# Hagtaril/HiddenPose

Hardware: AMD Instinct MI355X
Metric: samples/sec (128x128x512 meas) fwd+bwd (higher is better)
Workload: dtype f32; 1 GPU; NlosPose train step (fwd+L2Joint+BCEDice loss+bwd+Adam), 128x128x512 transients, batch 4/GPU, fp32, random-init weights, weight gradients of the 3^3 / 4^3 convolutions (and of small 1^3 ones) on a second stream; global_batch=4, world_size=1, parallelism=dp1

## Files before the change

### hiddenpose_amd/csrc/conv_kernels.hip

```cpp
#include <algorithm>
#include <cstdlib>
#include <cstring>
#include <mutex>
#include <type_traits>
#include <vector>

#include "hp_internal.h"

namespace hp {

using f32x16 = __attribute__((ext_vector_type(16))) float;
using bf16x8 = __attribute__((ext_vector_type(8))) __bf16;
using bf16x4 = __attribute__((ext_vector_type(4))) __bf16;
using bf16x2 = __attribute__((ext_vector_type(2))) __bf16;
using f32x2 = __attribute__((ext_vector_type(2))) float;
using s16x4 = __attribute__((ext_vector_type(4))) short;

__device__ __forceinline__ bf16x4 to_bf16x4(const float4 v) {
  const bf16x2 lo = __builtin_convertvector((f32x2){v.x, v.y}, bf16x2);
  const bf16x2 hi = __builtin_convertvector((f32x2){v.z, v.w}, bf16x2);
  return (bf16x4){lo[0], lo[1], hi[0], hi[1]};
}

enum IgemmMode { MODE_CONV = 0, MODE_DECONV = 1, MODE_DGRAD_S2K3 = 2, MODE_STEM = 3 };
// ... 2247 lines not shown
      const float* pl = ring + ((z + a - 3) & 7) * SF_PLANE + (2 * wave) * SF_RX + lane;
#pragma unroll
      for (int bb = 0; bb < 7; ++bb) {
        const float* wt = wl + ((a * 7 + bb) * 7) * 64 + sub * 16;
#pragma unroll
        for (int c = 0; c < 7; ++c) {
          float wr[16];
#pragma unroll
          for (int q = 0; q < 4; ++q) {
            const f32x4c t4 = *(const f32x4c*)(wt + c * 64 + 4 * q);
            wr[4 * q] = t4[0];
            wr[4 * q + 1] = t4[1];
            wr[4 * q + 2] = t4[2];
            wr[4 * q + 3] = t4[3];
          }
#pragma unroll
          for (int r = 0; r < 2; ++r) {
            const float xv = pl[(r + bb) * SF_RX + c];
#pragma unroll
            for (int cg = 0; cg < 16; ++cg) acc[r][cg] = __builtin_amdgcn_mfma_f32_4x4x1f32(wr[cg], xv, acc[r][cg], 0, 0, 0);
          }
        }
      }
    }
#pragma unroll
    for (int r = 0; r < 2; ++r) {
      const int oy = y0 + 2 * wave + r;
      const bool row_ok = oy < H;
      const long orow = (((long)b * D + z) * H + oy) * W + x0;
#pragma unroll
      for (int hh = 0; hh < 2; ++hh) {
#pragma unroll
        for (int cg = 0; cg < 8; ++cg)
#pragma unroll
          for (int i = 0; i < 4; ++i) ot[lane * 33 + cg * 4 + i] = acc[r][8 * hh + cg][i];
        if (row_ok) {
          if (stats && lane < 32) {
            float s = 0.f, q = 0.f;
            const int nv = min(64, W - x0);
            for (int v = 0; v < nv; ++v) {
              const float val = ot[v * 33 + lane];
              s += val;
              q += val * val;
            }
            ssum[hh] += s;
            ssq[hh] += q;
          }
          const int q4 = lane & 7;
#pragma unroll
          for (int it = 0; it < 8; ++it) {
            const int v = it * 8 + (lane >> 3);
            if (x0 + v < W) {
              const float* sp = ot + v * 33 + 4 * q4;
              *(float4*)(Y + (orow + v) * 64 + 32 * hh + 4 * q4) = make_float4(sp[0], sp[1], sp[2], sp[3]);
            }
          }
        }
      }
    }
    if (z + 1 < ze) stage_store(z + 4, nv);
    __syncthreads();
  }
  if (stats && lane < 32) {
#pragma unroll
    for (int hh = 0; hh < 2; ++hh) {
      double* const slot = stats + (size_t)(blockIdx.x & (HP_STATS_SLOTS - 1)) * 128;
      atomicAdd(slot + 32 * hh + lane, (double)ssum[hh]);
      atomicAdd(slot + 64 + 32 * hh + lane, (double)ssq[hh]);
    }
  }
}

__global__ void k_pack_weight(const float* __restrict__ w, float* __restrict__ out, int Cout, int Cin, int taps,
                              int transposed, int swap, int to_torch) {
  const long total = (long)Cout * Cin * taps;
  for (long i = (long)blockIdx.x * blockDim.x + threadIdx.x; i < total; i += (long)gridDim.x * blockDim.x) {
    const int inner = (int)(i % (swap ? Cout : Cin));
    long r = i / (swap ? Cout : Cin);
    const int outer = (int)(r % (swap ? Cin : Cout));
    const int t = (int)(r / (swap ? Cin : Cout));
    const int co = swap ? inner : outer, ci = swap ? outer : inner;
    const long ti = transposed ? ((long)ci * Cout + co) * taps + t : ((long)co * Cin + ci) * taps + t;
    if (to_torch)
      ((float*)w)[ti] = out[i];
    else
      out[i] = w[ti];
  }
}

__global__ __launch_bounds__(256) void k_pack_weight_tiled(const float* __restrict__ w, float* __restrict__ out, int Cout,
                                                           int Cin, int taps, int transposed, int swap, int to_torch,
                                                           int out_half = 0) {
  __shared__ float tile[64][65];
  const int A = swap ? Cin : Cout, Bn = swap ? Cout : Cin;
  const int a = blockIdx.y, bn0 = blockIdx.x * 64;
  const int nb = min(64, Bn - bn0), n = nb * taps;
  auto torch_index = [&](int bn, int t) -> long {
    const int co = swap ? bn : a, ci = swap ? a : bn;
    return transposed ? ((long)ci * Cout + co) * taps + t : ((long)co * Cin + ci) * taps + t;
  };
  if (!to_torch) {
    for (int e = threadIdx.x; e < n; e += 256) {
      const int bl = e / taps, t = e - bl * taps;
      tile[bl][t] = w[torch_index(bn0 + bl, t)];
    }
    __syncthreads();
    for (int e = threadIdx.x; e < taps * 64; e += 256) {
      const int t = e >> 6, bl = e & 63;
      if (bl < nb) hp_st1(out, ((long)t * A + a) * Bn + bn0 + bl, tile[bl][t], out_half);
    }
  } else {
    for (int e = threadIdx.x; e < taps * 64; e += 256) {
      const int t = e >> 6, bl = e & 63;
      if (bl < nb) tile[bl][t] = out[((long)t * A + a) * Bn + bn0 + bl];
    }
    __syncthreads();
    for (int e = threadIdx.x; e < n; e += 256) {
      const int bl = e / taps, t = e - bl * taps;
      ((float*)w)[torch_index(bn0 + bl, t)] = tile[bl][t];
    }
  }
}

__global__ void k_pack_stem(const float* __restrict__ w, float* __restrict__ out, int Cout, int kpad, int to_torch) {
  const long total = (long)Cout * kpad;
  for (long i = (long)blockIdx.x * blockDim.x + threadIdx.x; i < total; i += (long)gridDim.x * blockDim.x) {
    const int k = (int)(i % kpad), n = (int)(i / kpad);
    if (to_torch) {
      if (k < 343) ((float*)w)[(long)n * 343 + k] = out[i];
    } else {
      out[i] = k < 343 ? w[(long)n * 343 + k] : 0.f;
    }
  }
}

struct ConvPlan {
  IgemmGeom fwd, dgrad, wgrad;
  int fwd_classes = 1, dgrad_classes = 1, wgrad_tapsum = 1;
  bool stem = false, dgrad_zero_fill = false;
  int planes = 0;
};

static void set_shifts(IgemmGeom& g) {
  g.sw = g.sh = g.sd = -1;
  if (g.mode >= 0 && is_pow2(g.gw) && is_pow2(g.gh) && is_pow2(g.gd) && g.M < (1l << 32)) {
    g.sw = ilog2(g.gw);
    g.sh = ilog2(g.gh);
    g.sd = ilog2(g.gd);
  }
}

static int make_plan(const hp_conv_desc& d, ConvPlan& p) {
  HP_REQUIRE(d.B >= 1 && d.Cin >= 1 && d.Cout >= 1, "conv: bad channel/batch sizes");
  HP_REQUIRE(d.precision >= HP_PRECISION_FP32 && d.precision <= HP_PRECISION_BF16X6, "conv: unknown precision %d", d.precision);
  HP_REQUIRE(d.io == 0 || d.precision == HP_PRECISION_BF16, "conv: bf16 activation tensors (io = %d) go with HP_PRECISION_BF16", d.io);
  p.planes = d.precision;
  const int k = d.k, s = d.stride, pad = d.pad;
  IgemmGeom f{};
  if (!d.transposed) {
    const int Do = (d.Di + 2 * pad - k) / s + 1, Ho = (d.Hi + 2 * pad - k) / s + 1, Wo = (d.Wi + 2 * pad - k) / s + 1;
    p.stem = (d.Cin == 1 && k == 7 && s == 1 && pad == 3);
    if (!p.stem) HP_REQUIRE(d.Cin % 4 == 0, "conv: Cin must be a multiple of 4 (got %d)", d.Cin);
    HP_REQUIRE(s == 1 || s == 2, "conv: stride must be 1 or 2");
    const int kpt = p.stem ? (343 + 31) / 32 : (d.Cin + 31) / 32;
    f = IgemmGeom{p.stem ? MODE_STEM : MODE_CONV, d.B, d.Di, d.Hi, d.Wi, d.Cin, Do, Ho, Wo, d.Cout, Do, Ho, Wo, 1,
                  k, s, pad, 0, (long)d.B * Do * Ho * Wo, kpt};
    p.fwd = f;
    p.fwd_classes = 1;
    p.wgrad = f;
    p.wgrad_tapsum = p.stem ? 1 : k * k * k;
    IgemmGeom g{};
    if (p.stem) {
      g = IgemmGeom{MODE_CONV, d.B, Do, Ho, Wo, d.Cout, d.Di, d.Hi, d.Wi, 1, d.Di, d.Hi, d.Wi, 1,
                    7, 1, 3, 1, (long)d.B * d.Di * d.Hi * d.Wi, d.Cout / 32};
      p.dgrad_classes = 1;
    } else if (s == 1) {
      HP_REQUIRE(d.Cout % 4 == 0, "conv dgrad: Cout must be a multiple of 4 (got %d)", d.Cout);
      g = IgemmGeom{MODE_CONV, d.B, Do, Ho, Wo, d.Cout, d.Di, d.Hi, d.Wi, d.Cin, d.Di, d.Hi, d.Wi, 1,
                    k, 1, pad, 1, (long)d.B * d.Di * d.Hi * d.Wi, (d.Cout + 31) / 32};
      p.dgrad_classes = 1;
    } else if (k == 3 && pad == 1) {
      HP_REQUIRE(d.Di % 2 == 0 && d.Hi % 2 == 0 && d.Wi % 2 == 0 && d.Cout % 32 == 0, "conv dgrad s2: even dims needed");
      g = IgemmGeom{MODE_DGRAD_S2K3, d.B, Do, Ho, Wo, d.Cout, d.Di, d.Hi, d.Wi, d.Cin, d.Di / 2, d.Hi / 2, d.Wi / 2, 2,
                    3, 1, 1, 0, (long)d.B * (d.Di / 2) * (d.Hi / 2) * (d.Wi / 2), d.Cout / 32};
      p.dgrad_classes = 8;
    } else if (k == 1 && pad == 0) {
      HP_REQUIRE(d.Di % 2 == 0 && d.Hi % 2 == 0 && d.Wi % 2 == 0 && d.Cout % 32 == 0, "conv dgrad s2: even dims needed");
      g = IgemmGeom{MODE_CONV, d.B, Do, Ho, Wo, d.Cout, d.Di, d.Hi, d.Wi, d.Cin, Do, Ho, Wo, 2,
                    1, 1, 0, 0, (long)d.B * Do * Ho * Wo, d.Cout / 32};
      p.dgrad_classes = 1;
      p.dgrad_zero_fill = true;
    } else {
      set_error("conv: unsupported stride-2 kernel %d pad %d", k, pad);
      return HP_ERR_UNSUPPORTED;
    }
    p.dgrad = g;
  } else {
    HP_REQUIRE(k == 4 && s == 2 && pad == 1, "deconv: only k4 s2 p1 is supported");
    HP_REQUIRE(d.Cin % 32 == 0 && d.Cout % 32 == 0, "deconv: channels must be multiples of 32");
    const int Do = 2 * d.Di, Ho = 2 * d.Hi, Wo = 2 * d.Wi;
    f = IgemmGeom{MODE_DECONV, d.B, d.Di, d.Hi, d.Wi, d.Cin, Do, Ho, Wo, d.Cout, d.Di, d.Hi, d.Wi, 2,
                  4, 1, 1, 0, (long)d.B * d.Di * d.Hi * d.Wi, d.Cin / 32};
    p.fwd = f;
    p.fwd_classes = 8;
    p.wgrad = f;
    p.wgrad_tapsum = 64;
    p.dgrad = IgemmGeom{MODE_CONV, d.B, Do, Ho, Wo, d.Cout, d.Di, d.Hi, d.Wi, d.Cin, d.Di, d.Hi, d.Wi, 1,
                        4, 2, 1, 0, (long)d.B * d.Di * d.Hi * d.Wi, d.Cout / 32};
    p.dgrad_classes = 1;
  }
  HP_REQUIRE((long)d.B * d.Di * d.Hi * d.Wi * (d.transposed ? 8 : 1) < (1l << 31), "conv: more than 2^31 voxels per tensor");
  set_shifts(p.fwd);
  set_shifts(p.dgrad);
  set_shifts(p.wgrad);
  p.fwd.welems = p.wgrad.welems = p.stem ? (long)d.Cout * ((343 + 31) / 32 * 32) : (long)d.Cout * d.Cin * k * k * k;
  p.dgrad.welems = (long)d.Cout * d.Cin * k * k * k;
  return HP_OK;
}

template <bool STEM, bool STATS, int NP, bool XH = false>
static void launch_igemm_bn(const IgemmGeom& g, int classes, const void* X, const float* W, const float* bias, void* Y,
                            double* stats, const void* addend, const unsigned char* amask, hipStream_t st) {
  if constexpr (NP == 1 && !STEM && !XH) {
    if (g.xh && g.Cin % 64 == 0) return launch_igemm_bn<STEM, STATS, NP, true>(g, classes, X, W, bias, Y, stats, addend, amask, st);
  }
  const unsigned mt = (unsigned)((g.M + BM - 1) / BM);
  static const bool gl_on = !(getenv("HP_IGEMM_GL") && atoi(getenv("HP_IGEMM_GL")) == 0);
  const bool gl = XH && g.wh && gl_on;
  static const bool bl_on = !(getenv("HP_IGEMM_BL") && atoi(getenv("HP_IGEMM_BL")) == 0);
  const bool bl = !XH && !g.xh && !g.wh && !STEM && bl_on && g.Cin % 32 == 0 && (long)g.Nout * g.Cin * class_ntaps(g, 0) * 4 * (g.mode == MODE_DECONV ? 8 : 1) < (1l << 31);
  static const bool slab_on = !(getenv("HP_IGEMM_SLAB") && atoi(getenv("HP_IGEMM_SLAB")) == 0);
  if (slab_on && g.Nout <= 64) {
    IgemmGeom gs = g;
    gs.slab = (int)((mt + 7) / 8);
    const dim3 grid((mt + 7) / 8 * 8, 1, classes);
    if constexpr (!XH && !STEM) {
      if (bl && g.Nout > 32) {
        hipLaunchKernelGGL((k_igemm<64, false, STATS, NP, false, false, true>), grid, dim3(CT), 0, st, X, W, bias, Y, stats, addend, amask, gs);
        return;
      }
    }
  }
  if (g.Nout > 64) {
    const unsigned tn = (unsigned)((g.Nout + 127) / 128);
    IgemmGeom gg = g;
    gg.tn = tn > 1 ? (int)tn : 0;
    gg.slab = slab_on ? (int)((mt + 7) / 8) : 0;
    const dim3 grid = (tn > 1 || gg.slab) ? dim3((mt + 7) / 8 * 8 * (tn > 1 ? tn : 1), 1, classes) : dim3(mt, 1, classes);
    if constexpr (XH) {
      if (gl) {
        hipLaunchKernelGGL((k_igemm<128, STEM, STATS, NP, true, true>), grid, dim3(CT), 0, st, X, W, bias, Y, stats, addend, amask, gg);
        return;
      }
    }
    if constexpr (!XH && !STEM) {
      if (bl) {
        hipLaunchKernelGGL((k_igemm<128, false, STATS, NP, false, false, true>), grid, dim3(CT), 0, st, X, W, bias, Y, stats, addend, amask, gg);
        return;
      }
    }
    hipLaunchKernelGGL((k_igemm<128, STEM, STATS, NP, XH>), grid, dim3(CT), 0, st, X, W, bias, Y, stats, addend, amask, gg);
  } else if (g.Nout > 32) {
    if constexpr (XH) {
      if (gl) {
        hipLaunchKernelGGL((k_igemm<64, STEM, STATS, NP, true, true>), dim3(mt, 1, classes), dim3(CT), 0, st, X, W, bias, Y, stats, addend, amask, g);
        return;
      }
    }
    if constexpr (!XH && !STEM) {
      if (bl) {
        hipLaunchKernelGGL((k_igemm<64, false, STATS, NP, false, false, true>), dim3(mt, 1, classes), dim3(CT), 0, st, X, W, bias, Y, stats, addend, amask, g);
        return;
      }
    }
    hipLaunchKernelGGL((k_igemm<64, STEM, STATS, NP, XH>), dim3(mt, 1, classes), dim3(CT), 0, st, X, W, bias, Y, stats, addend, amask, g);
  } else {
    hipLaunchKernelGGL((k_igemm<32, STEM, STATS, NP, XH>), dim3(mt, 1, classes), dim3(CT), 0, st, X, W, bias, Y, stats, addend, amask, g);
  }
}

template <int NP>
static void launch_igemm_p(const IgemmGeom& g, int classes, bool stem, const void* X, const float* W, const float* bias,
                           void* Y, double* stats, const void* addend, const unsigned char* amask, hipStream_t st) {
  if (stem) {
    if (stats) launch_igemm_bn<true, true, NP>(g, classes, X, W, bias, Y, stats, addend, amask, st);
    else launch_igemm_bn<true, false, NP>(g, classes, X, W, bias, Y, stats, addend, amask, st);
  } else {
    if (stats) launch_igemm_bn<false, true, NP>(g, classes, X, W, bias, Y, stats, addend, amask, st);
    else launch_igemm_bn<false, false, NP>(g, classes, X, W, bias, Y, stats, addend, amask, st);
  }
}

static void launch_igemm(const IgemmGeom& g, int classes, bool stem, int planes, const void* X, const float* W,
                         const float* bias, void* Y, double* stats, const void* addend, hipStream_t st,
                         const unsigned char* amask = nullptr) {
  switch (planes) {
    case 1: launch_igemm_p<1>(g, classes, stem, X, W, bias, Y, stats, addend, amask, st); break;
    case 2: launch_igemm_p<2>(g, classes, stem, X, W, bias, Y, stats, addend, amask, st); break;
    case 3: launch_igemm_p<3>(g, classes, stem, X, W, bias, Y, stats, addend, amask, st); break;
    default: launch_igemm_p<0>(g, classes, stem, X, W, bias, Y, stats, addend, amask, st); break;
  }
}

}

using namespace hp;

extern "C" size_t hp_conv3d_packed_weight_elems(const hp_conv_desc* d) {
  if (!d) return 0;
  if (!d->transposed && d->Cin == 1 && d->k == 7) return (size_t)d->Cout * ((343 + 31) / 32 * 32);
  return (size_t)d->Cout * d->Cin * d->k * d->k * d->k;
}

extern "C" int hp_conv3d_pack_weight(const hp_conv_desc* d, const float* w_torch, void* w_fwd_v, void* w_dgrad_v,
                                     void* stream) {
  float* const w_fwd = (float*)w_fwd_v;
  float* const w_dgrad = (float*)w_dgrad_v;
  HP_REQUIRE(d && w_torch, "hp_conv3d_pack_weight: null argument");
  ConvPlan p;
  int rc = make_plan(*d, p);
  if (rc) return rc;
  hipStream_t st = (hipStream_t)stream;
  const int taps = d->k * d->k * d->k;
  if (p.stem) {
    const int kpad = p.fwd.kpt * BK;
    HP_PROF("conv_pack_weight", st);
    if (w_fwd) hipLaunchKernelGGL(k_pack_stem, dim3(64), dim3(256), 0, st, w_torch, w_fwd, d->Cout, kpad, 0);
    if (w_dgrad) hipLaunchKernelGGL(k_pack_weight, dim3(64), dim3(256), 0, st, w_torch, w_dgrad, d->Cout, 1, 343, 0, 1, 0);
  } else {
    HP_REQUIRE(taps <= 64, "conv: at most 64 taps (got %d)", taps);
    HP_PROF("conv_pack_weight", st);
    const int wh = (d->io & HP_IO_W_BF16) ? 1 : 0;
    if (w_fwd)
      hipLaunchKernelGGL(k_pack_weight_tiled, dim3((d->Cin + 63) / 64, d->Cout), dim3(256), 0, st, w_torch, w_fwd, d->Cout,
                         d->Cin, taps, d->transposed, 0, 0, wh);
    if (w_dgrad)
      hipLaunchKernelGGL(k_pack_weight_tiled, dim3((d->Cout + 63) / 64, d->Cin), dim3(256), 0, st, w_torch, w_dgrad, d->Cout,
                         d->Cin, taps, d->transposed, 1, 0, wh);
  }
  HP_CHECK_HIP(hipGetLastError());
  return HP_OK;
}

extern "C" int hp_conv3d_unpack_wgrad(const hp_conv_desc* d, const float* dw_packed, float* dw_torch, void* stream) {
  HP_REQUIRE(d && dw_packed && dw_torch, "hp_conv3d_unpack_wgrad: null argument");
  ConvPlan p;
  int rc = make_plan(*d, p);
  if (rc) return rc;
  hipStream_t st = (hipStream_t)stream;
  const int taps = d->k * d->k * d->k;
  HP_PROF("conv_pack_weight", st);
  if (p.stem) {
    hipLaunchKernelGGL(k_pack_stem, dim3(64), dim3(256), 0, st, dw_torch, (float*)dw_packed, d->Cout, p.fwd.kpt * BK, 1);
  } else {
    hipLaunchKernelGGL(k_pack_weight_tiled, dim3((d->Cin + 63) / 64, d->Cout), dim3(256), 0, st, dw_torch, (float*)dw_packed,
                       d->Cout, d->Cin, taps, d->transposed, 0, 1);
  }
  HP_CHECK_HIP(hipGetLastError());
  return HP_OK;
}

extern "C" int hp_conv3d_forward(const hp_conv_desc* d, const void* x, const float* w_fwd, const float* bias, void* y,
                                 double* stats, void* stream) {
  HP_REQUIRE(d && x && w_fwd && y, "hp_conv3d_forward: null argument");
  ConvPlan p;
  int rc = make_plan(*d, p);
  if (rc) return rc;
  HP_REQUIRE(!(p.stem && (d->io & HP_IO_X_BF16)), "hp_conv3d_forward: the stem reads its single-channel input as fp32");
  p.fwd.xh = (d->io & HP_IO_X_BF16) ? 1 : 0;
  p.fwd.yh = (d->io & HP_IO_Y_BF16) ? 1 : 0;
  p.fwd.wh = (d->io & HP_IO_W_BF16) ? 1 : 0;
  HP_REQUIRE(!p.fwd.wh || (p.fwd.xh && p.planes == 1 && !p.stem && d->Cin % 64 == 0),
             "hp_conv3d_forward: bf16 packed weights go with a bf16 input, HP_PRECISION_BF16 and Cin %% 64 == 0");
  hipStream_t st = (hipStream_t)stream;
  if (stats) HP_CHECK_HIP(hipMemsetAsync(stats, 0, sizeof(double) * 2 * d->Cout * HP_STATS_SLOTS, st));
  if (p.stem && p.planes == 1 && d->Cout == 64 && !bias && !p.fwd.yh) {
    const int pz = (d->Di + SFH_TZ - 1) / SFH_TZ, py = (d->Hi + SFH_TY - 1) / SFH_TY, px = (d->Wi + SFH_TX - 1) / SFH_TX;
    const long tiles = (long)d->B * pz * py * px;
    const int per_wg = (int)std::max<long>(1, (tiles + 511) / 512);
    const size_t lds = sizeof(__bf16) * (SFH_W + 4 * SFH_COPY) + sizeof(float) * 8 * 64 * 2;
    static std::once_flag lds_once_h;
    static hipError_t lds_rc_h = hipSuccess;
    std::call_once(lds_once_h, [&] {
      lds_rc_h = hipFuncSetAttribute((const void*)k_stem_fwd_bf16, hipFuncAttributeMaxDynamicSharedMemorySize, (int)lds);
    });
    HP_CHECK_HIP(lds_rc_h);
    HP_PROF("conv_igemm_stem", st);
    hipLaunchKernelGGL(k_stem_fwd_bf16, dim3((unsigned)((tiles + per_wg - 1) / per_wg)), dim3(512), lds, st, (const float*)x, w_fwd,
                       (float*)y, stats, d->Di, d->Hi, d->Wi, p.fwd.kpt * BK, pz, py, px, tiles, per_wg);
  } else if (p.stem && p.planes == 0 && d->Cout == 64 && !bias && !p.fwd.yh) {
    const int tiles_x = (d->Wi + SF_TX - 1) / SF_TX, tiles_y = (d->Hi + SF_TY - 1) / SF_TY;
    const long cols = (long)tiles_x * tiles_y * d->B;
    int zsplit = (int)std::max<long>(1, std::min<long>((d->Di + 15) / 16, (1024 + cols - 1) / cols));
    const int zchunk = (d->Di + zsplit - 1) / zsplit;
    zsplit = (d->Di + zchunk - 1) / zchunk;
    const size_t lds = sizeof(float) * (343 * 64 + 8 * SF_PLANE + 4 * 64 * 33);
    static std::once_flag lds_once;
    static hipError_t lds_rc = hipSuccess;
    std::call_once(lds_once, [&] {
      lds_rc = hipFuncSetAttribute((const void*)k_stem_fwd_mfma, hipFuncAttributeMaxDynamicSharedMemorySize, (int)lds);
    });
    HP_CHECK_HIP(lds_rc);
    HP_PROF("conv_igemm_stem", st);
    hipLaunchKernelGGL(k_stem_fwd_mfma, dim3((unsigned)(tiles_x * tiles_y * zsplit), (unsigned)d->B), dim3(256), lds, st,
                       (const float*)x, w_fwd, (float*)y, stats, d->Di, d->Hi, d->Wi, p.fwd.kpt * BK, tiles_x, tiles_y, zchunk);
  } else {
    HP_PROF(p.stem ? "conv_igemm_stem" : d->transposed ? "conv_igemm_deconv" : d->k == 1 ? "conv_igemm_k1" : "conv_igemm_k3", st);
    launch_igemm(p.fwd, p.fwd_classes, p.stem, p.planes, x, w_fwd, bias, y, stats, nullptr, st);
  }
  HP_CHECK_HIP(hipGetLastError());
  return HP_OK;
}

extern "C" int hp_linear_forward(const float* x, const float* w, const float* bias, const float* addend, float* y, long M, int K,
                                 int N, int precision, void* stream) {
  HP_REQUIRE(x && w && y && M >= 1 && M < (1l << 31) && K >= 4 && N >= 1, "hp_linear_forward: bad argument");
  hp_conv_desc d{1, 1, 1, (int)M, K, N, 1, 1, 0, 0, precision, 0};
  ConvPlan p;
  int rc = make_plan(d, p);
  if (rc) return rc;
  hipStream_t st = (hipStream_t)stream;
  {
    HP_PROF("linear_fwd", st);
    launch_igemm(p.fwd, 1, false, p.planes, x, w, bias, y, nullptr, addend, st);
  }
  HP_CHECK_HIP(hipGetLastError());
  return HP_OK;
}

extern "C" int hp_linear_geglu_forward(const float* x, const float* w, const float* bias, float* y, long M, int K,
                                       int N2, int precision, void* stream) {
  HP_REQUIRE(x && w && y && M >= 1 && M < (1l << 31) && K >= 4, "hp_linear_geglu_forward: bad argument");
  HP_REQUIRE(N2 >= 128 && N2 % 128 == 0, "hp_linear_geglu_forward: 2 * hidden must be a multiple of 128 (got %d)", N2);
  hp_conv_desc d{1, 1, 1, (int)M, K, N2, 1, 1, 0, 0, precision, 0};
  ConvPlan p;
  int rc = make_plan(d, p);
  if (rc) return rc;
  p.fwd.geglu = 1;
  hipStream_t st = (hipStream_t)stream;
  {
    HP_PROF("linear_fwd", st);
    launch_igemm(p.fwd, 1, false, p.planes, x, w, bias, y, nullptr, nullptr, st);
  }
  HP_CHECK_HIP(hipGetLastError());
  return HP_OK;
}

static bool launch_igemm_bns(const IgemmGeom& g, const void* X, const float* W, void* Y, const void* addend,
                             const unsigned char* amask, hipStream_t st) {
  const bool dense_out = g.os == 1 && g.gd == g.Do && g.gh == g.Ho && g.gw == g.Wo;
  if (g.mode != MODE_CONV || !dense_out || g.M % BM != 0 || g.Nout <= 32 || g.Nout % (g.Nout > 64 ? 128 : 64) != 0 || g.xh || g.yh ||
      g.wh || g.ah)
    return false;
  const unsigned mt = (unsigned)(g.M / BM);
  static const bool bl_on = !(getenv("HP_IGEMM_BL") && atoi(getenv("HP_IGEMM_BL")) == 0);
  static const bool slab_on = !(getenv("HP_IGEMM_SLAB") && atoi(getenv("HP_IGEMM_SLAB")) == 0);
  const bool bl = bl_on && g.Cin % 32 == 0 && (long)g.Nout * g.Cin * class_ntaps(g, 0) * 4 < (1l << 31);
  IgemmGeom gg = g;
  gg.slab = slab_on ? (int)((mt + 7) / 8) : 0;
#define HP_BNS_LAUNCH(BN_, BL_)                                                                                                     \
  do {                                                                                                                             \
    if (g.bn_mask)                                                                                                                 \
      hipLaunchKernelGGL((k_igemm<BN_, false, false, 0, false, false, BL_, 2>), grid, dim3(CT), 0, st, X, W, nullptr, Y, nullptr,   \
                         addend, amask, gg);                                                                                       \
    else                                                                                                                           \
      hipLaunchKernelGGL((k_igemm<BN_, false, false, 0, false, false, BL_, 1>), grid, dim3(CT), 0, st, X, W, nullptr, Y, nullptr,   \
                         addend, amask, gg);                                                                                       \
  } while (0)
  if (g.Nout <= 64) {
    const dim3 grid = gg.slab ? dim3((mt + 7) / 8 * 8, 1, 1) : dim3(mt, 1, 1);
    if (bl) HP_BNS_LAUNCH(64, true);
    else HP_BNS_LAUNCH(64, false);
    return true;
  }
  const unsigned tn = (unsigned)(g.Nout / 128);
  gg.tn = tn > 1 ? (int)tn : 0;
  const dim3 grid = (tn > 1 || gg.slab) ? dim3((mt + 7) / 8 * 8 * (tn > 1 ? tn : 1), 1, 1) : dim3(mt, 1, 1);
  if (bl) HP_BNS_LAUNCH(128, true);
  else HP_BNS_LAUNCH(128, false);
#undef HP_BNS_LAUNCH
  return true;
}

extern "C" int hp_conv3d_backward_data_bnsums(const hp_conv_desc* d, const void* dy, const float* w_dgrad, void* dx, const void* addend,
                                              const unsigned char* addend_mask, const float* z, const float* mean,
                                              const float* rstd, const float* gamma, const float* beta, int relu,
                                              const unsigned char* relu_mask, double* sums, int* fused, void* stream) {
  HP_REQUIRE(d && dy && w_dgrad && dx && z && mean && rstd && sums && fused && (!relu || relu_mask || (gamma && beta)),
             "hp_conv3d_backward_data_bnsums: null argument");
  *fused = 0;
  ConvPlan p;
  int rc = make_plan(*d, p);
  if (rc) return rc;
  hipStream_t st = (hipStream_t)stream;
  if (p.planes == 0 && !p.stem && !p.dgrad_zero_fill && d->io == 0 && p.dgrad_classes == 1 &&
      (!addend_mask || (addend && d->Cin % 4 == 0 && d->Cin > 32))) {
    IgemmGeom g = p.dgrad;
    g.bn_z = z;
    g.bn_mean = mean;
    g.bn_rstd = rstd;
    g.bn_gamma = gamma;
    g.bn_beta = beta;
    g.bn_sums = sums;
    g.bn_relu = relu ? 1 : 0;
    g.bn_mask = relu ? relu_mask : nullptr;
    HP_CHECK_HIP(hipMemsetAsync(sums, 0, sizeof(double) * 2 * g.Nout * HP_STATS_SLOTS, st));
    HP_PROF("conv_igemm_dgrad", st);
    if (launch_igemm_bns(g, dy, w_dgrad, dx, addend, addend_mask, st)) {
      HP_CHECK_HIP(hipGetLastError());
      *fused = 1;
      return HP_OK;
    }
  }
  return hp_conv3d_backward_data_masked(d, dy, w_dgrad, dx, addend, addend_mask, stream);
}

extern "C" int hp_conv3d_backward_data(const hp_conv_desc* d, const void* dy, const float* w_dgrad, void* dx,
                                       const void* addend, void* stream) {
  return hp_conv3d_backward_data_masked(d, dy, w_dgrad, dx, addend, nullptr, stream);
}

extern "C" int hp_conv3d_backward_data_masked(const hp_conv_desc* d, const void* dy, const float* w_dgrad, void* dx,
                                              const void* addend, const unsigned char* addend_mask, void* stream) {
  HP_REQUIRE(d && dy && w_dgrad && dx, "hp_conv3d_backward_data: null argument");
  ConvPlan p;
  int rc = make_plan(*d, p);
  if (rc) return rc;
  const int dyh = (d->io & HP_IO_DY_BF16) ? 1 : 0, dxh = (d->io & HP_IO_DX_BF16) ? 1 : 0;
  HP_REQUIRE(!(p.stem && (dyh || dxh)), "hp_conv3d_backward_data: the stem's data gradient is fp32 in, fp32 out");
  p.dgrad.xh = dyh;
  p.dgrad.yh = p.dgrad.ah = dxh;
  p.dgrad.wh = (d->io & HP_IO_W_BF16) ? 1 : 0;
  HP_REQUIRE(!p.dgrad.wh || (dyh && p.planes == 1 && !p.stem && p.dgrad.Cin % 64 == 0),
             "hp_conv3d_backward_data: bf16 packed weights go with a bf16 dy, HP_PRECISION_BF16 and Cout %% 64 == 0");
  const size_t esz = dxh ? 2 : 4;
  HP_REQUIRE(!addend_mask || (addend && !p.stem && !p.dgrad_zero_fill && d->Cin % 4 == 0 && d->Cin > 32),
             "hp_conv3d_backward_data_masked: a masked addend needs a dense data gradient with > 32 input channels, a multiple of 4");
  hipStream_t st = (hipStream_t)stream;
  if (p.stem) {
    HP_REQUIRE(d->Cout == 64, "stem data gradient: 64 output channels expected (got %d)", d->Cout);
    HP_REQUIRE((long)d->Hi * d->Wi <= (1l << 21), "stem data gradient: H * W up to 2^21 (31-bit offsets inside a 4-plane dZ tile), got %d x %d", d->Hi, d->Wi);
    const size_t nb = sizeof(float) * (size_t)d->B * d->Di * d->Hi * d->Wi;
    if (addend) HP_CHECK_HIP(hipMemcpyAsync(dx, addend, nb, hipMemcpyDeviceToDevice, st));
    else HP_CHECK_HIP(hipMemsetAsync(dx, 0, nb, st));
    const int pz = (d->Di + SP_Z - 1) / SP_Z, py = (d->Hi + SP_Y - 1) / SP_Y, px = (d->Wi + SP_X - 1) / SP_X;
    HP_PROF("conv_stem_dgrad", st);
    const long cols = (long)py * px * d->B;
    int zsplit = 1;
    long best = -1;
    for (int zs = 1; zs <= std::min(pz, 32); ++zs) {
      const long cost = ((cols * zs + 767) / 768) * ((pz + zs - 1) / zs + 2);
      if (best < 0 || cost < best) best = cost, zsplit = zs;
    }
    if (const char* e = getenv("HP_STEM_DGRAD_ZSPLIT")) zsplit = std::max(1, std::min(pz, atoi(e)));
    const int zchunk = (pz + zsplit - 1) / zsplit;
    zsplit = (pz + zchunk - 1) / zchunk;
    hipLaunchKernelGGL(p.planes == 1 ? k_stem_dgrad<true> : k_stem_dgrad<false>, dim3((unsigned)(py * px * zsplit), (unsigned)d->B), dim3(CT), 0,
                       st, (const float*)dy, w_dgrad, (float*)dx, d->Di, d->Hi, d->Wi, pz, py, px, zchunk);
    HP_CHECK_HIP(hipGetLastError());
    return HP_OK;
  }
  if (p.dgrad_zero_fill) {
    const size_t nb = esz * (size_t)d->B * d->Di * d->Hi * d->Wi * d->Cin;
    if (addend == dx) {}
    else if (addend) HP_CHECK_HIP(hipMemcpyAsync(dx, addend, nb, hipMemcpyDeviceToDevice, st));
    else HP_CHECK_HIP(hipMemsetAsync(dx, 0, nb, st));
  }
  {
    HP_PROF("conv_igemm_dgrad", st);
    launch_igemm(p.dgrad, p.dgrad_classes, false, p.planes, dy, w_dgrad, nullptr, dx, nullptr, addend, st, addend_mask);
  }
  HP_CHECK_HIP(hipGetLastError());
  return HP_OK;
}

struct WgradSplit {
  int TT, tap_groups, tiles_c, tiles_total;
  bool multitap;
  long msplit;
};
static WgradSplit wgrad_split(const ConvPlan& p) {
  const IgemmGeom& g = p.wgrad;
  const int Kc = p.stem ? g.kpt * BK : g.Cin;
  WgradSplit w{};
  w.TT = (g.Nout >= 128 && Kc >= 128) ? 128 : 64;
  w.multitap = !p.stem && w.TT == 64 && g.mode == MODE_CONV && g.k == 3;
  w.tap_groups = w.multitap ? (27 + 3) / 4 : p.wgrad_tapsum;
  const int tiles_n = (g.Nout + w.TT - 1) / w.TT;
  w.tiles_c = (Kc + w.TT - 1) / w.TT;
  const long base_blocks = (long)tiles_n * w.tiles_c * w.tap_groups;
  long hi = std::max<long>(1, (4096 + base_blocks - 1) / base_blocks);
  hi = std::min<long>(std::min<long>(hi, std::max<long>(1, g.M / (4 * WG_KM))), 4096);
  static const int fixed_env = getenv("HP_WGRAD_R0") ? atoi(getenv("HP_WGRAD_R0")) : -1;
  const long r0 = fixed_env >= 0 ? fixed_env : ((g.xh && g.yh) ? 768 : 96);
  long best = hi;
  struct Memo { long M, base, r0, hi, best; };
  static std::mutex memo_mu;
  static std::vector<Memo> memo;
  bool known = false;
  {
    std::lock_guard<std::mutex> lk(memo_mu);
    for (const Memo& m : memo)
      if (m.M == g.M && m.base == base_blocks && m.r0 == r0 && m.hi == hi) {
        best = m.best;
        known = true;
        break;
      }
  }
  if (r0 > 0 && !known) {
    const long slots = 768;
    auto cost = [&](long ms) {
      const long rows = ((g.M + ms - 1) / ms + WG_KM - 1) / WG_KM * WG_KM;
      const long blocks = base_blocks * ms;
      double c = (double)((blocks + slots - 1) / slots) * (double)(rows + r0);
      if (blocks & 7) c *= 1.02;
      return c;
    };
    double cmin = cost(hi);
    for (long ms = 1; ms < hi; ++ms) cmin = std::min(cmin, cost(ms));
    for (long ms = hi; ms >= 1; --ms)
      if (cost(ms) <= 1.03 * cmin) {
        best = ms;
        break;
      }
  }
  for (; !known;) {
    const long chunk = ((g.M + best - 1) / best + WG_KM - 1) / WG_KM * WG_KM;
    const long need = (g.M + chunk - 1) / chunk;
    if (need >= best) break;
    best = need;
  }
  if (!known) {
    std::lock_guard<std::mutex> lk(memo_mu);
    if (memo.size() < 4096) memo.push_back({g.M, base_blocks, r0, hi, best});
  }
  w.msplit = best;
  w.tiles_total = tiles_n * w.tiles_c;
  return w;
}

extern "C" int hp_conv3d_backward_weight_split(const hp_conv_desc* d, long* msplit, long* chunk_rows) {
  HP_REQUIRE(d && msplit && chunk_rows, "hp_conv3d_backward_weight_split: null argument");
  ConvPlan p;
  int rc = make_plan(*d, p);
  if (rc) return rc;
  p.wgrad.xh = (d->io & HP_IO_X_BF16) ? 1 : 0;
  p.wgrad.yh = (d->io & HP_IO_DY_BF16) ? 1 : 0;
  const WgradSplit ws = wgrad_split(p);
  *msplit = ws.msplit;
  *chunk_rows = ((p.wgrad.M + ws.msplit - 1) / ws.msplit + WG_KM - 1) / WG_KM * WG_KM;
  return HP_OK;
}

extern "C" int hp_conv3d_backward_weight(const hp_conv_desc* d, const void* x, const void* dy, float* dw_packed,
                                         void* stream) {
  HP_REQUIRE(d && x && dy && dw_packed, "hp_conv3d_backward_weight: null argument");
  ConvPlan p;
  int rc = make_plan(*d, p);
  if (rc) return rc;
  hipStream_t st = (hipStream_t)stream;
  const int xh = (d->io & HP_IO_X_BF16) ? 1 : 0, dyh = (d->io & HP_IO_DY_BF16) ? 1 : 0;
  HP_REQUIRE(!(p.stem && xh), "hp_conv3d_backward_weight: the stem reads its single-channel input as fp32");
  p.wgrad.xh = xh;
  p.wgrad.yh = dyh;
  const IgemmGeom& g = p.wgrad;
  const int Kc = p.stem ? g.kpt * BK : g.Cin;
  HP_CHECK_HIP(hipMemsetAsync(dw_packed, 0, sizeof(float) * hp_conv3d_packed_weight_elems(d), st));
  if (p.stem && p.planes <= 1 && d->Cout == 64 && !dyh) {
    const int pz = (d->Di + SP_Z - 1) / SP_Z, py = (d->Hi + SP_Y - 1) / SP_Y, px = (d->Wi + SP_X - 1) / SP_X;
    const long tiles = (long)d->B * pz * py * px;
    const int per_wg = (int)std::max<long>(1, (tiles + 1023) / 1024);
    HP_PROF("conv_wgrad", st);
    hipLaunchKernelGGL(p.planes == 1 ? k_stem_wgrad_bf16 : k_stem_wgrad_full, dim3((unsigned)((tiles + per_wg - 1) / per_wg)), dim3(256),
                       0, st, (const float*)x, (const float*)dy, dw_packed, d->Di,
                       d->Hi, d->Wi, pz, py, px, tiles, per_wg, Kc);
    HP_CHECK_HIP(hipGetLastError());
    return HP_OK;
  }
  if (!p.stem && p.planes == 0 && !xh && !dyh && g.mode == MODE_CONV && g.k == 1 && g.s == 1 && g.os == 1 && g.M >= (1l << 16)) {
    const bool wide_n = g.Nout % 256 == 0 && g.Cin == 64, wide_c = g.Nout == 64 && g.Cin % 256 == 0;
    if (wide_n || wide_c) {
      const int tiles = wide_n ? g.Nout / 256 : g.Cin / 256;
      long ms = std::max<long>(1, std::min<long>(1024 / tiles, g.M / (4 * WG_KM)));
      ms = std::max<long>(8, ms / 8 * 8);
      HP_PROF("conv_wgrad", st);
      if (wide_n)
        hipLaunchKernelGGL((k_wgrad_dense<256, 64>), dim3((unsigned)(tiles * ms)), dim3(CT), 0, st, (const float*)x, (const float*)dy, dw_packed, g.M, g.Nout,
                           g.Cin, (int)ms, 1);
      else
        hipLaunchKernelGGL((k_wgrad_dense<64, 256>), dim3((unsigned)(tiles * ms)), dim3(CT), 0, st, (const float*)x, (const float*)dy, dw_packed, g.M, g.Nout,
                           g.Cin, (int)ms, tiles);
      HP_CHECK_HIP(hipGetLastError());
      return HP_OK;
// ... 85 lines not shown
```

### hiddenpose_amd/csrc/hp_internal.h

```cpp
#pragma once
#include <hip/hip_runtime.h>

#include "hp_host.h"

namespace hp {

#define HP_CHECK_HIP(expr)                                                              \
  do {                                                                                  \
    hipError_t _e = (expr);                                                             \
    if (_e != hipSuccess) {                                                             \
      ::hp::set_error("%s:%d: %s -> %s", __FILE__, __LINE__, #expr, hipGetErrorString(_e)); \
      return HP_ERR_HIP;                                                                \
    }                                                                                   \
  } while (0)

struct ProfScope {
  ProfScope(const char* name, hipStream_t st);
  ~ProfScope();
  int slot = -1;
  hipStream_t st = nullptr;
  hipEvent_t stop = nullptr;
};
#define HP_PROF(name, stream) ::hp::ProfScope _hp_prof_scope(name, stream)

constexpr int ATTN_JOINT_SPLITS = 32;
constexpr int ATTN_GROUPED_MAX_N = 64;
constexpr int ATTN_BWD_DQ_SPLITS = 32;
void launch_attn_bwd_joint_keys(const float* ws_dk, const float* ws_dv, float* dK, float* dV, int BH, int Ntok, int dh, int nj, int frames,
                                hipStream_t st);
void launch_attn_bwd_dq_joint(const float* Q, const float* K0, const float* V, const float* dout, const float* lse, const float* delta,
                              float* part, float* dQ, int BH, int heads, int dh, int Ntok, int nj, hipStream_t st);
void launch_attention_patch(const float* Q, const float* K, const float* V, float* out, float* lse, int B, int heads, int dh, int Ntok,
                            int nj, int n, int frames, hipStream_t st);
void launch_attention_joint_merge(const float* part, float* out, float* lse, int BH, int heads, int dh, int Ntok, int nj, int nsplit,
                                  hipStream_t st);
void launch_attn_bwd_delta(const float* out, const float* dout, float* delta, int B, int heads, int dh, int Ntok, hipStream_t st);
void launch_attn_bwd_dq_patch(const float* Q, const float* K, const float* V, const float* dout, const float* lse, const float* delta,
                              float* dQ, int BH, int heads, int dh, int Ntok, int nj, int n, int frames, hipStream_t st);
void launch_attn_bwd_dq_joint_merge(const float* part, float* dQ, int BH, int Ntok, int dh, int nj, int nsplit, hipStream_t st);
void launch_attention_patch16(const float* Q, const float* K, const float* V, float* out, float* lse, int B, int heads, int dh, int Ntok,
                              int nj, int n, int frames, int precision, hipStream_t st);
void launch_attn_bwd_dq_joint_masked(const float* Q, const float* K0, const float* V, const float* dout, const float* lse,
                                     const float* delta, float* part, float* dQ, int BH, int heads, int dh, int Ntok, int nj,
                                     const unsigned char* key_mask, hipStream_t st);
inline int attn_masked16_check(const char* who, int num_joints, int mask_patch_queries) {
  HP_REQUIRE(mask_patch_queries == 0 || mask_patch_queries == 1, "%s: mask_patch_queries must be 0 or 1", who);
  if (mask_patch_queries) {
    set_error("%s: mask_patch_queries 1 not built at a 16-bit precision (only the joint / class queries apply the mask there)", who);
    return HP_ERR_UNSUPPORTED;
  }
  if (num_joints == 0) {
    set_error("%s: num_joints 0 not built (with no joint / class key an all-masked group would have an empty key set)", who);
    return HP_ERR_UNSUPPORTED;
  }
  return HP_OK;
}

#ifdef __HIPCC__
__device__ __forceinline__ float4 hp_ld4(const void* p, long i, int half) {
  if (half) {
    const uint2 u = *reinterpret_cast<const uint2*>(reinterpret_cast<const unsigned short*>(p) + i);
    return make_float4(__uint_as_float(u.x << 16), __uint_as_float(u.x & 0xffff0000u), __uint_as_float(u.y << 16),
                       __uint_as_float(u.y & 0xffff0000u));
  }
  return *reinterpret_cast<const float4*>(reinterpret_cast<const float*>(p) + i);
}
__device__ __forceinline__ float hp_ld1(const void* p, long i, int half) {
  if (half) return __uint_as_float((unsigned)reinterpret_cast<const unsigned short*>(p)[i] << 16);
  return reinterpret_cast<const float*>(p)[i];
}
__device__ __forceinline__ unsigned short hp_f2bf(float v) {
  typedef __attribute__((ext_vector_type(2))) float hp_f32x2;
  typedef __attribute__((ext_vector_type(2))) __bf16 hp_bf16x2;
  const hp_bf16x2 h = __builtin_convertvector((hp_f32x2){v, 0.f}, hp_bf16x2);
  return __builtin_bit_cast(unsigned int, h) & 0xffffu;
}
__device__ __forceinline__ void hp_st4(void* p, long i, float4 v, int half) {
  if (half) {
    typedef __attribute__((ext_vector_type(2))) float hp_f32x2;
    typedef __attribute__((ext_vector_type(2))) __bf16 hp_bf16x2;
    const hp_bf16x2 lo = __builtin_convertvector((hp_f32x2){v.x, v.y}, hp_bf16x2);
    const hp_bf16x2 hi = __builtin_convertvector((hp_f32x2){v.z, v.w}, hp_bf16x2);
    *reinterpret_cast<uint2*>(reinterpret_cast<unsigned short*>(p) + i) =
        make_uint2(__builtin_bit_cast(unsigned int, lo), __builtin_bit_cast(unsigned int, hi));
    return;
  }
  *reinterpret_cast<float4*>(reinterpret_cast<float*>(p) + i) = v;
}
__device__ __forceinline__ unsigned hp_extent(long total, long base_off, int esz) {
  const long bytes = (total - base_off) * esz;
  return bytes >= 0x80000000l ? 0x80000000u : bytes > 0 ? (unsigned)bytes : 0u;
}
__device__ __forceinline__ void hp_st1(void* p, long i, float v, int half) {
  if (half) reinterpret_cast<unsigned short*>(p)[i] = hp_f2bf(v);
  else reinterpret_cast<float*>(p)[i] = v;
}
#endif

}
```

Measured before the change: 8.742 samples/s.

## Add 32x32 MFMA fp32 stem forward kernel variants and make it default

Adds a new 7^3 single-channel stem forward kernel built on 32x32x2 f32 MFMA instead of the existing 4x4 MFMA path. It uses a ring of staged input planes in LDS, prefetches the next z-plane into registers while computing, and pairs taps across the two half-waves. Three tile variants can be chosen through an environment variable, with the 32x32 column variant as the default. The aim is higher matrix-core throughput for the stem convolution, at the cost of more LDS, register pressure and a new code path that must get edges and stats right.

```diff
diff --git a/hiddenpose_amd/csrc/conv_kernels.hip b/hiddenpose_amd/csrc/conv_kernels.hip
--- a/hiddenpose_amd/csrc/conv_kernels.hip
+++ b/hiddenpose_amd/csrc/conv_kernels.hip
@@ -2573,6 +2573,15 @@
   }
 }
 
+static int stem_fwd_variant() {
+  const char* const e = getenv("HP_STEM_FWD_KERNEL");
+  if (!e || !*e || !strcmp(e, "32x32")) return STEM_FWD32_COLS4;
+  if (!strcmp(e, "4x4")) return -1;
+  if (!strcmp(e, "32x32w8")) return STEM_FWD32_COLS8;
+  if (!strcmp(e, "32x32r")) return STEM_FWD32_ROWS4;
+  return -2;
+}
+
 }
 
 using namespace hp;
@@ -2645,6 +2654,8 @@
              "hp_conv3d_forward: bf16 packed weights go with a bf16 input, HP_PRECISION_BF16 and Cin %% 64 == 0");
   hipStream_t st = (hipStream_t)stream;
   if (stats) HP_CHECK_HIP(hipMemsetAsync(stats, 0, sizeof(double) * 2 * d->Cout * HP_STATS_SLOTS, st));
+  const bool stem_fp32 = p.stem && p.planes == 0 && d->Cout == 64 && !bias && !p.fwd.yh;
+  const int stem32 = stem_fp32 ? stem_fwd_variant() : -1;
   if (p.stem && p.planes == 1 && d->Cout == 64 && !bias && !p.fwd.yh) {
     const int pz = (d->Di + SFH_TZ - 1) / SFH_TZ, py = (d->Hi + SFH_TY - 1) / SFH_TY, px = (d->Wi + SFH_TX - 1) / SFH_TX;
     const long tiles = (long)d->B * pz * py * px;
@@ -2659,7 +2670,12 @@
     HP_PROF("conv_igemm_stem", st);
     hipLaunchKernelGGL(k_stem_fwd_bf16, dim3((unsigned)((tiles + per_wg - 1) / per_wg)), dim3(512), lds, st, (const float*)x, w_fwd,
                        (float*)y, stats, d->Di, d->Hi, d->Wi, p.fwd.kpt * BK, pz, py, px, tiles, per_wg);
-  } else if (p.stem && p.planes == 0 && d->Cout == 64 && !bias && !p.fwd.yh) {
+  } else if (stem32 != -1) {
+    HP_REQUIRE(stem32 >= 0, "hp_conv3d_forward: HP_STEM_FWD_KERNEL is 4x4, 32x32, 32x32w8 or 32x32r");
+    HP_PROF("conv_igemm_stem", st);
+    rc = launch_stem_fwd32(stem32, (const float*)x, w_fwd, (float*)y, stats, d->B, d->Di, d->Hi, d->Wi, p.fwd.kpt * BK, st);
+    if (rc) return rc;
+  } else if (stem_fp32) {
     const int tiles_x = (d->Wi + SF_TX - 1) / SF_TX, tiles_y = (d->Hi + SF_TY - 1) / SF_TY;
     const long cols = (long)tiles_x * tiles_y * d->B;
     int zsplit = (int)std::max<long>(1, std::min<long>((d->Di + 15) / 16, (1024 + cols - 1) / cols));
diff --git a/hiddenpose_amd/csrc/hp_internal.h b/hiddenpose_amd/csrc/hp_internal.h
--- a/hiddenpose_amd/csrc/hp_internal.h
+++ b/hiddenpose_amd/csrc/hp_internal.h
@@ -56,6 +56,14 @@
   return HP_OK;
 }
 
+enum {
+  STEM_FWD32_COLS4 = 0,
+  STEM_FWD32_COLS8 = 1,
+  STEM_FWD32_ROWS4 = 2,
+};
+int launch_stem_fwd32(int variant, const float* x, const float* w_fwd, float* y, double* stats, int B, int D, int H, int W,
+                      int kpad, hipStream_t st);
+
 #ifdef __HIPCC__
 __device__ __forceinline__ float4 hp_ld4(const void* p, long i, int half) {
   if (half) {
diff --git a/hiddenpose_amd/csrc/stem_fwd_kernels.hip b/hiddenpose_amd/csrc/stem_fwd_kernels.hip
--- /dev/null
+++ b/hiddenpose_amd/csrc/stem_fwd_kernels.hip
@@ -0,0 +1,305 @@
+#include <algorithm>
+#include <mutex>
+#include <type_traits>
+
+#include "hp_internal.h"
+
+namespace hp {
+
+namespace {
+
+constexpr int S32_TY = 8, S32_TX = 64, S32_RY = S32_TY + 6, S32_RX = 72, S32_PLANE = S32_RY * S32_RX;
+constexpr int S32_SLOTS = 344;
+constexpr int S32_ZPAD = 160;
+using f32x16s = __attribute__((ext_vector_type(16))) float;
+
+template <int ROWS, bool CH_ROWS>
+__global__ __launch_bounds__(64 * (S32_TY / ROWS), CH_ROWS ? 1 : 2) void k_stem_fwd32(const float* __restrict__ X, const float* __restrict__ Wp,
+                                                                    float* __restrict__ Y, double* __restrict__ stats, int D, int H,
+                                                                    int W, int kpad, int tiles_x, int tiles_y, int zchunk) {
+  constexpr int NW = S32_TY / ROWS, NT = 64 * NW;
+  extern __shared__ __attribute__((aligned(16))) float s32_smem[];
+  float* const wl = s32_smem;
+  float* const ring = wl + S32_SLOTS * 64;
+  float* const red = ring + 8 * S32_PLANE;
+  float* const zpad = red + NW * 64 * 2;
+  const int tid = threadIdx.x, lane = tid & 63, wave = tid >> 6, col = lane & 31, half = lane >> 5;
+  int t_ = blockIdx.x;
+  const int bx = t_ % tiles_x;
+  t_ /= tiles_x;
+  const int by = t_ % tiles_y;
+  const int bz = t_ / tiles_y;
+  const int b = blockIdx.y;
+  const int x0 = bx * S32_TX, y0 = by * S32_TY;
+  const int zb = bz * zchunk, ze = min(D, zb + zchunk);
+  const float* xb = X + (long)b * D * H * W;
+
+  for (int e = tid; e < S32_SLOTS * 64; e += NT) {
+    const int tap = e >> 6;
+    wl[e] = tap < 343 ? Wp[(long)(e & 63) * kpad + tap] : 0.f;
+  }
+  for (int e = tid; e < S32_ZPAD; e += NT) zpad[e] = 0.f;
+  constexpr int SK = (S32_PLANE + NT - 1) / NT;
+  int soff[SK];
+  unsigned smask = 0;
+#pragma unroll
+  for (int k = 0; k < SK; ++k) {
+    const int e = tid + NT * k;
+    const int ly = e / S32_RX, lx = e - ly * S32_RX;
+    const int yy = y0 + ly - 3, xx = x0 + lx - 3;
+    const bool ok = e < S32_PLANE && lx < S32_TX + 6 && (unsigned)yy < (unsigned)H && (unsigned)xx < (unsigned)W;
+    soff[k] = ok ? yy * W + xx : 0;
+    smask |= ok ? (1u << k) : 0u;
+  }
+  auto stage_load = [&](int zin, float (&v)[SK]) {
+    const bool zok = (unsigned)zin < (unsigned)D;
+    const float* src = xb + (long)(zok ? zin : 0) * H * W;
+#pragma unroll
+    for (int k = 0; k < SK; ++k) v[k] = (zok && ((smask >> k) & 1u)) ? src[soff[k]] : 0.f;
+  };
+  auto stage_store = [&](int zin, const float (&v)[SK]) {
+    float* dst = ring + (zin & 7) * S32_PLANE + tid;
+#pragma unroll
+    for (int k = 0; k < SK; ++k)
+      if (tid + NT * k < S32_PLANE) dst[NT * k] = v[k];
+  };
+  if (zb < ze)
+    for (int zin = zb - 3; zin <= zb + 3; ++zin) {
+      float v[SK];
+      stage_load(zin, v);
+      stage_store(zin, v);
+    }
+  __syncthreads();
+
+  const int vox_off = (wave * ROWS) * S32_RX + col;
+  const float* const wlane = wl + half * 64 + col;
+  const bool full_x = x0 + S32_TX <= W;
+
+  float ssum = 0.f, ssq = 0.f;
+  f32x16s rsum[2], rsq[2];
+  if constexpr (CH_ROWS) {
+#pragma unroll
+    for (int nt = 0; nt < 2; ++nt)
+#pragma unroll
+      for (int g = 0; g < 16; ++g) rsum[nt][g] = rsq[nt][g] = 0.f;
+  }
+
+  for (int z = zb; z < ze; ++z) {
+    float nv[SK];
+    if (z + 1 < ze) stage_load(z + 4, nv);
+    __builtin_amdgcn_sched_barrier(0);
+    f32x16s acc[ROWS][2][2];
+#pragma unroll
+    for (int r = 0; r < ROWS; ++r)
+#pragma unroll
+      for (int xh = 0; xh < 2; ++xh)
+#pragma unroll
+        for (int nt = 0; nt < 2; ++nt)
+#pragma unroll
+          for (int g = 0; g < 16; ++g) acc[r][xh][nt][g] = 0.f;
+
+    struct Frag {
+      float xv[ROWS][2], wv[2];
+    };
+    auto kload = [&](Frag& f, const float* vp, const float* wp) {
+#pragma unroll
+      for (int nt = 0; nt < 2; ++nt) f.wv[nt] = wp[32 * nt];
+#pragma unroll
+      for (int r = 0; r < ROWS; ++r)
+#pragma unroll
+        for (int xh = 0; xh < 2; ++xh) f.xv[r][xh] = vp[r * S32_RX + 32 * xh];
+      __builtin_amdgcn_sched_barrier(0);
+    };
+    auto kmma = [&](const Frag& f) {
+#pragma unroll
+      for (int r = 0; r < ROWS; ++r)
+#pragma unroll
+        for (int xh = 0; xh < 2; ++xh)
+#pragma unroll
+          for (int nt = 0; nt < 2; ++nt) {
+            if constexpr (CH_ROWS)
+              acc[r][xh][nt] = __builtin_amdgcn_mfma_f32_32x32x2f32(f.wv[nt], f.xv[r][xh], acc[r][xh][nt], 0, 0, 0);
+            else
+              acc[r][xh][nt] = __builtin_amdgcn_mfma_f32_32x32x2f32(f.xv[r][xh], f.wv[nt], acc[r][xh][nt], 0, 0, 0);
+          }
+    };
+    auto plane = [&](int a) { return ring + ((z + a - 3) & 7) * S32_PLANE + vox_off; };
+    Frag cur, nxt;
+    auto plane_pair = [&](int ap, auto last) __attribute__((always_inline)) {
+      constexpr int NS = decltype(last)::value ? 25 : 49;
+      const float* const pe = plane(2 * ap);
+      const float* const po = plane(2 * ap + 1);
+      const float* const wt = wlane + ap * (49 * 128);
+      auto pair = [&](const float* pl, int u) { return pl + (u % 7 < 6 ? half : half * (S32_RX - 6)) + (u / 7) * S32_RX + u % 7; };
+      const float* const cross = half ? (decltype(last)::value ? zpad + col : po) : pe + 6 * S32_RX + 6;
+#pragma unroll
+      for (int i = 0; i < NS; ++i) {
+        cur = nxt;
+        const int n = i + 1;
+        if (n < 24) kload(nxt, pair(pe, 2 * n), wt + n * 128);
+        else if (n == 24) kload(nxt, cross, wt + n * 128);
+        else if (n < NS) kload(nxt, pair(po, 2 * (n - 25) + 1), wt + n * 128);
+        else if (!decltype(last)::value) kload(nxt, plane(2 * ap + 2) + half, wt + n * 128);
+        kmma(cur);
+      }
+    };
+    kload(nxt, plane(0) + half, wlane);
+#pragma unroll 1
+    for (int ap = 0; ap < 3; ++ap) plane_pair(ap, std::false_type{});
+    plane_pair(3, std::true_type{});
+    if (z + 1 < ze) stage_store(z + 4, nv);
+
+    if constexpr (!CH_ROWS) {
+#pragma unroll
+      for (int r = 0; r < ROWS; ++r) {
+        const int oy = y0 + wave * ROWS + r;
+        if (oy < H) {
+          float s = 0.f, q = 0.f;
+#pragma unroll
+          for (int xh = 0; xh < 2; ++xh) {
+            const int xl = x0 + 32 * xh + 4 * half;
+            float* const yo = Y + ((((long)b * D + z) * H + oy) * W + xl) * 64 + col;
+#pragma unroll
+            for (int qd = 0; qd < 4; ++qd) {
+              float lo[4], hi[4];
+#pragma unroll
+              for (int j = 0; j < 4; ++j) {
+                const int xo = 8 * qd + j;
+                const bool ok = full_x || xl + xo < W;
+                const float v0 = acc[r][xh][0][4 * qd + j], v1 = acc[r][xh][1][4 * qd + j];
+                if (ok) {
+                  yo[xo * 64] = v0;
+                  yo[xo * 64 + 32] = v1;
+                }
+                if (stats) {
+                  const float m0 = ok ? v0 : 0.f, m1 = ok ? v1 : 0.f;
+                  const float t0 = __shfl_xor(m0, 32), t1 = __shfl_xor(m1, 32);
+                  lo[j] = half ? t1 : m0;
+                  hi[j] = half ? m1 : t0;
+                }
+              }
+              if (stats) {
+#pragma unroll
+                for (int j = 0; j < 4; ++j) {
+                  s += lo[j];
+                  q = __builtin_fmaf(lo[j], lo[j], q);
+                }
+#pragma unroll
+                for (int j = 0; j < 4; ++j) {
+                  s += hi[j];
+                  q = __builtin_fmaf(hi[j], hi[j], q);
+                }
+              }
+            }
+          }
+          ssum += s;
+          ssq += q;
+        }
+      }
+    } else {
+#pragma unroll
+      for (int r = 0; r < ROWS; ++r) {
+        const int oy = y0 + wave * ROWS + r;
+        if (oy < H) {
+#pragma unroll
+          for (int xh = 0; xh < 2; ++xh) {
+            const int ox = x0 + 32 * xh + col;
+            if (ox < W) {
+              float* const yo = Y + ((((long)b * D + z) * H + oy) * W + ox) * 64 + 4 * half;
+#pragma unroll
+              for (int nt = 0; nt < 2; ++nt)
+#pragma unroll
+                for (int q = 0; q < 4; ++q) {
+                  const float4 v = make_float4(acc[r][xh][nt][4 * q], acc[r][xh][nt][4 * q + 1], acc[r][xh][nt][4 * q + 2],
+                                               acc[r][xh][nt][4 * q + 3]);
+                  *(float4*)(yo + 32 * nt + 8 * q) = v;
+                  rsum[nt][4 * q] += v.x;
+                  rsum[nt][4 * q + 1] += v.y;
+                  rsum[nt][4 * q + 2] += v.z;
+                  rsum[nt][4 * q + 3] += v.w;
+                  rsq[nt][4 * q] += v.x * v.x;
+                  rsq[nt][4 * q + 1] += v.y * v.y;
+                  rsq[nt][4 * q + 2] += v.z * v.z;
+                  rsq[nt][4 * q + 3] += v.w * v.w;
+                }
+            }
+          }
+        }
+      }
+    }
+    __syncthreads();
+  }
+
+  if (stats) {
+    if constexpr (!CH_ROWS) {
+      red[(wave * 64 + lane) * 2 + 0] = ssum;
+      red[(wave * 64 + lane) * 2 + 1] = ssq;
+    } else {
+#pragma unroll
+      for (int nt = 0; nt < 2; ++nt)
+#pragma unroll
+        for (int g = 0; g < 16; ++g) {
+          float sv = rsum[nt][g], qv = rsq[nt][g];
+#pragma unroll
+          for (int m = 1; m < 32; m <<= 1) {
+            sv += __shfl_xor(sv, m);
+            qv += __shfl_xor(qv, m);
+          }
+          if (col == 0) {
+            const int ch = 32 * nt + (g & 3) + 8 * (g >> 2) + 4 * half;
+            red[(wave * 64 + ch) * 2 + 0] = sv;
+            red[(wave * 64 + ch) * 2 + 1] = qv;
+          }
+        }
+    }
+    __syncthreads();
+    if (tid < 64) {
+      double sv = 0.0, qv = 0.0;
+#pragma unroll
+      for (int w = 0; w < NW; ++w) {
+        sv += (double)red[(w * 64 + tid) * 2 + 0];
+        qv += (double)red[(w * 64 + tid) * 2 + 1];
+      }
+      double* const slot = stats + (size_t)(blockIdx.x & (HP_STATS_SLOTS - 1)) * 128;
+      atomicAdd(slot + tid, sv);
+      atomicAdd(slot + 64 + tid, qv);
+    }
+  }
+}
+
+template <int ROWS, bool CH_ROWS>
+int launch_variant(const float* x, const float* w_fwd, float* y, double* stats, int B, int D, int H, int W, int kpad,
+                   hipStream_t st) {
+  constexpr int NW = S32_TY / ROWS;
+  const int tiles_x = (W + S32_TX - 1) / S32_TX, tiles_y = (H + S32_TY - 1) / S32_TY;
+  const long cols = (long)tiles_x * tiles_y * B;
+  int zsplit = (int)std::max<long>(1, std::min<long>((D + 15) / 16, (1024 + cols - 1) / cols));
+  const int zchunk = (D + zsplit - 1) / zsplit;
+  zsplit = (D + zchunk - 1) / zchunk;
+  const size_t lds = sizeof(float) * (S32_SLOTS * 64 + 8 * S32_PLANE + NW * 64 * 2 + S32_ZPAD);
+  static std::once_flag lds_once;
+  static hipError_t lds_rc = hipSuccess;
+  std::call_once(lds_once, [&] {
+    lds_rc = hipFuncSetAttribute((const void*)k_stem_fwd32<ROWS, CH_ROWS>, hipFuncAttributeMaxDynamicSharedMemorySize, (int)lds);
+  });
+  HP_CHECK_HIP(lds_rc);
+  hipLaunchKernelGGL((k_stem_fwd32<ROWS, CH_ROWS>), dim3((unsigned)(tiles_x * tiles_y * zsplit), (unsigned)B), dim3(64 * NW), lds, st,
+                     x, w_fwd, y, stats, D, H, W, kpad, tiles_x, tiles_y, zchunk);
+  return HP_OK;
+}
+
+}
+
+int launch_stem_fwd32(int variant, const float* x, const float* w_fwd, float* y, double* stats, int B, int D, int H, int W,
+                      int kpad, hipStream_t st) {
+  switch (variant) {
+    case STEM_FWD32_COLS4: return launch_variant<2, false>(x, w_fwd, y, stats, B, D, H, W, kpad, st);
+    case STEM_FWD32_COLS8: return launch_variant<1, false>(x, w_fwd, y, stats, B, D, H, W, kpad, st);
+    case STEM_FWD32_ROWS4: return launch_variant<2, true>(x, w_fwd, y, stats, B, D, H, W, kpad, st);
+    default: break;
+  }
+  set_error("launch_stem_fwd32: unknown variant %d", variant);
+  return HP_ERR_BAD_ARG;
+}
+
+}
```

Result: no change. 8.768 samples/s, median of 6 (+0.3%).
